# divideon/xvc

Measured on AMD Instinct MI355X. Metric: hot-path frame passes/s (TZ + sub-pel ME, MC, transform + RDOQ + dequant + inverse, deblock, pad, PSNR parts), bit-exact vs the reference's classes, higher is better.
Workload: dtype u16; 1 GPU; 1920x1080 yuv420p 30fps synthetic, QP 32, internal bitdepth 10, 16x16 CUs, TZ range 96, RDOQ (RdoQuant::QuantRdo + CoeffSignHideRdo, picture-initial CABAC contexts); cus_per_picture=8160, parallelism=3 independent picture chains in flight

## Files before the change

### xvc_amd/csrc/k_rdoq.h

```cpp
#ifndef XVCGPU_K_RDOQ_H_
#define XVCGPU_K_RDOQ_H_

#include "dev_common.h"
#include "k_me.h"
#include "k_me2.h"
#include "k_quant.h"
#include "k_rdoq4.h"
#include "k_rdoq_common.h"
#include "k_scan.h"
#include "xvcgpu_internal.h"


template <int G = 64, typename S, typename CF, typename LEV>
__device__ __forceinline__ int wave_rdoq(S &s, int lane, const BlockQuant &bq, int w, int h,
                                         bool luma, int scan_order, bool sign_hide,
                                         const xvcgpu_rdoq_contexts &ctx,
                                         const xvcgpu_rdoq_params &prm, CF cf, LEV lev,
                                         bool stage_ctx = true, bool clear_levels = true) {
  const int sbs = (w == 2 || h == 2) ? 1 : 2;
  const int sb_size = 1 << (2 * sbs);
  const int gw = w >> sbs, gh = h >> sbs;
  const int rw = w < 32 ? w : 32, rh = h < 32 ? h : 32;
  const int rgw = rw >> sbs, rgh = rh >> sbs;
  const int size_cls = (rq_log2(w) + rq_log2(h)) >> 1;
// ... 1307 lines not shown
struct RqGlobalLev {
  int16_t *p;
  int w;
  __device__ __forceinline__ int16_t *operator()(int x, int y) const { return p + y * w + x; }
  __device__ __forceinline__ void store4(int px, int y, const int v[4]) const {
    int16_t *o = p + y * w + px;
    if ((reinterpret_cast<uintptr_t>(o) & 7) == 0) {
      *reinterpret_cast<uint2 *>(o) =
          make_uint2((unsigned)(v[0] & 0xffff) | ((unsigned)v[1] << 16),
                     (unsigned)(v[2] & 0xffff) | ((unsigned)v[3] << 16));
    } else {
      o[0] = (int16_t)v[0]; o[1] = (int16_t)v[1]; o[2] = (int16_t)v[2]; o[3] = (int16_t)v[3];
    }
  }
};

template <int G, int NSB, bool FOUR>
__device__ __forceinline__ void quant_rdo_packed_wave(
    RdoqPackedLds<G, NSB> &sm, int wave, int bd, const xvcgpu_tx_block *blocks, const int *list,
    const int *count, const int16_t *coeffs, const uint32_t *d_off, int16_t *levels,
    int32_t *nnz_out, const xvcgpu_rdoq_contexts *rq_ctx, const xvcgpu_rdoq_params *rq_prm,
    xvcgpu_cu_info *cu_patch = nullptr) {
  constexpr int GROUPS = 64 / G;
  const int g = threadIdx.x / G, lane = threadIdx.x % G;
  const int slot = wave * GROUPS + g;
  RQ_TRACE(0);
  RQ_TRACE_RT(0);
  const int n_list = *count;
  if (wave * GROUPS >= n_list) return;
  const bool active = slot < n_list;
  const int bi = active ? list[slot] : 0;
  const xvcgpu_tx_block b = blocks[bi];
  const xvcgpu_rdoq_params prm = rq_prm[bi];
  const int w = b.w, h = b.h;
  const int rw = w < 32 ? w : 32, rh = h < 32 ? h : 32;
  const uint32_t off = d_off[bi];
  const int16_t *src = coeffs + off;
  int16_t *cf = sm.cf[g], *lv = sm.lv[g];
  constexpr int kCtxWords = (int)sizeof(xvcgpu_rdoq_contexts) / 4;
  const int ctx_wi = (int)threadIdx.x < kCtxWords ? (int)threadIdx.x : kCtxWords - 1;
  const uint32_t word_own = reinterpret_cast<const uint32_t *>(&rq_ctx[prm.ctx_index])[ctx_wi];
  RQ_TRACE(1);
  int16_t *dst = levels + off;
  const bool wide = w == rw && h == rh && ((w * h) & 7) == 0 &&
                    ((reinterpret_cast<uintptr_t>(src) | reinterpret_cast<uintptr_t>(dst)) & 15) == 0;
  const bool sb4 = !(w == 2 || h == 2);
  const int rgw4 = rw >> 2;
  auto tile_pos = [sb4, rgw4, rw](int x, int y) {
    return sb4 ? ((y >> 2) * rgw4 + (x >> 2)) * RQ_CF_STRIDE + (((y & 3) << 2) | (x & 3))
               : y * rw + x;
  };
  if (active) {
    if (wide && sb4) {
      for (int i = lane; i < (w * h) >> 3; i += G) {
        const uint4 v8 = reinterpret_cast<const uint4 *>(src)[i];
        const int y = (8 * i) / rw, x = 8 * i - y * rw;
        const int p0 = tile_pos(x, y), p1 = rw == 4 ? tile_pos(0, y + 1) : tile_pos(x + 4, y);
        *reinterpret_cast<uint2 *>(cf + p0) = make_uint2(v8.x, v8.y);
        *reinterpret_cast<uint2 *>(cf + p1) = make_uint2(v8.z, v8.w);
        if (!FOUR) {
          *reinterpret_cast<uint2 *>(lv + p0) = make_uint2(0, 0);
          *reinterpret_cast<uint2 *>(lv + p1) = make_uint2(0, 0);
        }
      }
    } else {
      for (int i = lane; i < rw * rh; i += G) {
        const int y = i / rw, x = i - y * rw;
        cf[tile_pos(x, y)] = src[y * w + x];
        if (!FOUR) lv[tile_pos(x, y)] = 0;
      }
    }
  }
  RdoqView v;
  v.wl = sm.wl[g];
  v.fcs = NSB == 64 ? sm.fcs : sm.sb_code_cost[g];
  v.sb_dcz = sm.sb_dcz[g];
  v.rate_up = sm.rate_up[g];
  v.sb_live = sm.sb_live[g];
  v.sb_code_cost = sm.sb_code_cost[g];
  v.csbf_bits = sm.csbf_bits[g];
  v.csbf = sm.csbf[g];
  v.sb_of_scan = sm.sb_of_scan[g];
  v.lp_bits = sm.lp_bits;
  v.ctx_bits = sm.ctx_bits;
  RQ_TRACE(2);
  bool pending = active;
  int nnz = 0;
  for (;;) {
    const unsigned long long todo = __ballot(pending);
    if (!todo) break;
    const int leader = __ffsll((long long)todo) - 1;
    const int cur = __shfl((int)prm.ctx_index, leader, 64);
    const int kw = __shfl(w, leader, 64), kh = __shfl(h, leader, 64);
    const int kqp = __shfl((int)b.qp, leader, 64);
    const int kluma = __shfl((int)(b.comp == 0), leader, 64);
    const int kflags = __shfl((int)b.intra_pic, leader, 64);
    const int kpf = __shfl((int)prm.flags, leader, 64);
    const long long klambda = __shfl(prm.lambda, leader, 64);
    wave_sync();
    {
      static_assert(RQ_CTX_WORDS <= 64, "one word of contexts per lane");
      const uint32_t *cw = reinterpret_cast<const uint32_t *>(&rq_ctx[cur]);
      const uint32_t word = (int)prm.ctx_index == cur ? word_own : cw[ctx_wi];
      if ((int)threadIdx.x < RQ_CTX_WORDS)
        rq_stage_word(kEntropyBits, word, sm.ctx_bits + 8 * threadIdx.x);
    }
    wave_sync();
    RQ_TRACE(3);
    const bool take = pending && (int)prm.ctx_index == cur && w == kw && h == kh &&
                      (int)b.qp == kqp && (int)(b.comp == 0) == kluma &&
                      (int)b.intra_pic == kflags && (int)prm.flags == kpf &&
                      prm.lambda == klambda;
    if (take) {
      const int uw = __builtin_amdgcn_readfirstlane(w), uh = __builtin_amdgcn_readfirstlane(h);
      const int uqp = __builtin_amdgcn_readfirstlane((int)b.qp);
      const int uluma = __builtin_amdgcn_readfirstlane((int)(b.comp == 0));
      const int uflags = __builtin_amdgcn_readfirstlane((int)b.intra_pic);
      const int upf = __builtin_amdgcn_readfirstlane((int)prm.flags);
      const unsigned ulam_lo = (unsigned)__builtin_amdgcn_readfirstlane((int)(unsigned)prm.lambda);
      const unsigned ulam_hi = (unsigned)__builtin_amdgcn_readfirstlane(
          (int)(unsigned)((unsigned long long)prm.lambda >> 32));
      const long long ulambda = (long long)(((unsigned long long)ulam_hi << 32) | ulam_lo);
      const bool usb4 = !(uw == 2 || uh == 2);
      const int urw = uw < 32 ? uw : 32, urgw4 = urw >> 2;
      auto utile = [usb4, urgw4, urw](int x, int y) {
        return usb4 ? ((y >> 2) * urgw4 + (x >> 2)) * RQ_CF_STRIDE + (((y & 3) << 2) | (x & 3))
                    : y * urw + x;
      };
      xvcgpu_rdoq_params uprm = prm;
      uprm.lambda = ulambda;
      uprm.flags = (uint8_t)upf;
      const TxBlockFlags ufl = tx_block_flags(uflags);
      const int uscan = ufl.scan_order;
      const bool ush = ufl.sign_hide;
      auto ubq = [&](int bw, int bh) { return block_quant(bw, bh, uqp, bd, ufl.intra_pic); };
      auto cf_at = [cf, utile](int x, int y) { return (int)cf[utile(x, y)]; };
      auto lv_at = [lv, utile](int x, int y) { return lv + utile(x, y); };
      if (FOUR) {
        const RqTileCf cf4 = {cf, urgw4};
        const RqGlobalLev lv4 = {dst, uw};
        nnz = wave_rdoq4<G, 1>(v, lane, ubq(uw, uh), uw, uh, uluma != 0, ush, uprm, cf4, lv4);
      } else if (NSB == 64) {
        const BlockQuant q = ubq(uw, uh);
        if (rq4_takes(64, uw, uh, uscan))
          nnz = wave_rdoq4<64, 4>(v, lane, q, uw, uh, uluma != 0, ush, uprm, cf_at, lv_at);
        else
          nnz = wave_rdoq<G>(v, lane, q, uw, uh, uluma != 0, uscan, ush, rq_ctx[cur], uprm, cf_at,
                             lv_at, false, false);
      } else if (G == 16 && NSB == 16 && uw == 16 && uh == 16) {
        auto cf16 = [cf](int x, int y) {
          return (int)cf[((y >> 2) * 4 + (x >> 2)) * RQ_CF_STRIDE + (((y & 3) << 2) | (x & 3))];
        };
        auto lv16 = [lv](int x, int y) {
          return lv + ((y >> 2) * 4 + (x >> 2)) * RQ_CF_STRIDE + (((y & 3) << 2) | (x & 3));
        };
        nnz = wave_rdoq<G>(v, lane, ubq(16, 16), 16, 16, uluma != 0, uscan, ush, rq_ctx[cur], uprm,
                           cf16, lv16, false, false);
      } else {
        nnz = wave_rdoq<G>(v, lane, ubq(uw, uh), uw, uh, uluma != 0, uscan, ush, rq_ctx[cur], uprm,
                           cf_at, lv_at, false, false);
      }
      pending = false;
    }
  }
  wave_sync();
// ... 89 lines not shown
```

### xvc_amd/csrc/k_rdoq4.h

```cpp
#ifndef XVCGPU_K_RDOQ4_H_
#define XVCGPU_K_RDOQ4_H_

#include "dev_common.h"
#include "k_me2.h"
#include "k_quant.h"
#include "k_rdoq_common.h"
#include "k_scan.h"

template <int I>
__device__ __forceinline__ int rq4_quad_bcast(int v) {
  return __builtin_amdgcn_update_dpp(0, v, I * 0x55, 0xF, 0xF, false);
}
__device__ __forceinline__ int rq4_quad_or(int v) {
  v |= lane_xor<1>(v);
  v |= lane_xor<2>(v);
  return v;
}
__device__ __forceinline__ int rq4_quad_min(int v) {
  int o = lane_xor<1>(v);
  v = o < v ? o : v;
  o = lane_xor<2>(v);
  return o < v ? o : v;
}
__device__ __forceinline__ int rq4_quad_max(int v) {
// ... 26 lines not shown
  }
  return v;
}
template <int G>
__device__ __forceinline__ int rq4_sum(int v) {
  v = dpp_group_sum<16>(v);
  if (G == 64)
    v = __builtin_amdgcn_readlane(v, 0) + __builtin_amdgcn_readlane(v, 16) +
        __builtin_amdgcn_readlane(v, 32) + __builtin_amdgcn_readlane(v, 48);
  return v;
}
template <int G>
__device__ __forceinline__ unsigned rq4_wave_or8(unsigned v, int bits) {
  if (G == 64) {
    int o = rq4_quad_or((int)v);
    o |= rq4_row_half_mirror(o);
    o |= rq4_row_mirror(o);
    return (unsigned)(__builtin_amdgcn_readlane(o, 0) | __builtin_amdgcn_readlane(o, 16) |
                      __builtin_amdgcn_readlane(o, 32) | __builtin_amdgcn_readlane(o, 48));
  }
  unsigned r = 0;
  for (int b = 0; b < bits; b++) r |= (__ballot((v >> b) & 1u) ? 1u : 0u) << b;
  return r;
}
__device__ __forceinline__ long long rq4_readlane_i64(long long v, int l) {
  const unsigned lo = (unsigned)__builtin_amdgcn_readlane((int)(unsigned)v, l);
  const unsigned hi = (unsigned)__builtin_amdgcn_readlane((int)(v >> 32), l);
  return (long long)(((unsigned long long)hi << 32) | lo);
}
__device__ __forceinline__ long long rq4_add_wrap(long long a, long long b) {
  return (long long)((unsigned long long)a + (unsigned long long)b);
}
template <int G>
__device__ __forceinline__ long long rq4_sum_i64(long long v) {
  v = rq_group_sum_i64<16>(v);
  if (G == 64)
    v = rq4_add_wrap(rq4_add_wrap(rq4_readlane_i64(v, 0), rq4_readlane_i64(v, 16)),
                     rq4_add_wrap(rq4_readlane_i64(v, 32), rq4_readlane_i64(v, 48)));
  return v;
}
__device__ __forceinline__ unsigned rq4_row_scan_u32(unsigned v) {
  v += (unsigned)__builtin_amdgcn_update_dpp(0, (int)v, 0x111, 0xF, 0xF, true);
  v += (unsigned)__builtin_amdgcn_update_dpp(0, (int)v, 0x112, 0xF, 0xF, true);
  v += (unsigned)__builtin_amdgcn_update_dpp(0, (int)v, 0x114, 0xF, 0xF, true);
  v += (unsigned)__builtin_amdgcn_update_dpp(0, (int)v, 0x118, 0xF, 0xF, true);
  return v;
}
template <int S>
__device__ __forceinline__ long long rq4_xor_i64(long long v) {
  const int lo = lane_xor<S>((int)(unsigned)v), hi = lane_xor<S>((int)(v >> 32));
  return (long long)(((unsigned long long)(unsigned)hi << 32) | (unsigned)lo);
}
template <int G>
__device__ __forceinline__ long long rq4_suffix_i64(long long v) {
  const long long inc = rq_row_scan_i64(v);
  const long long row = rq_group_sum_i64<16>(v);
  long long behind = rq4_add_wrap(row - inc, v);
  if (G == 64) {
    const long long t1 = rq4_readlane_i64(row, 16), t2 = rq4_readlane_i64(row, 32),
                    t3 = rq4_readlane_i64(row, 48);
    const int r = ME2_LANE >> 4;
    behind = rq4_add_wrap(behind, r == 0 ? rq4_add_wrap(rq4_add_wrap(t1, t2), t3)
                                         : (r == 1 ? rq4_add_wrap(t2, t3) : (r == 2 ? t3 : 0ll)));
  }
  return behind;
}

__device__ __forceinline__ int rq4_sb_scan_index(int gw, int gh, int sx, int sy) {
  const int s = sx + sy, a = gw < gh ? gw : gh, b = gw < gh ? gh : gw;
  int t;
  if (s <= a) {
    t = (s * (s + 1)) >> 1;
  } else if (s <= b) {
    t = ((a * (a + 1)) >> 1) + (s - a) * a;
  } else {
    const int m = gw + gh - 1 - s;
    t = gw * gh - ((m * (m + 1)) >> 1);
  }
  return t + ((s < gh - 1 ? s : gh - 1) - sy);
}

__device__ __forceinline__ bool rq4_takes(int G, int w, int h, int scan_order) {
  const int rw = w < 32 ? w : 32, rh = h < 32 ? h : 32;
  return scan_order == 0 && w >= 4 && h >= 4 && (G == 64 || (rw >> 2) * (rh >> 2) * 4 <= G);
}
__device__ __forceinline__ bool rq4_needs_nr4(int w, int h) {
  const int rw = w < 32 ? w : 32, rh = h < 32 ? h : 32;
  return (rw >> 2) * (rh >> 2) > 16;
}

template <typename CF>
__device__ __forceinline__ auto rq4_load_row(const CF &cf, int px, int y, int c[4])
    -> decltype(cf.row4(px, y, c), void()) {
  cf.row4(px, y, c);
}
template <typename CF, typename... Dummy>
__device__ __forceinline__ void rq4_load_row(const CF &cf, int px, int y, int c[4], Dummy...) {
#pragma unroll
  for (int i = 0; i < 4; i++) c[i] = cf(px + i, y);
}
template <typename LEV>
__device__ __forceinline__ auto rq4_store_row(const LEV &lev, int px, int y, const int v[4])
    -> decltype(lev.store4(px, y, v), void()) {
  lev.store4(px, y, v);
}
template <typename LEV, typename... Dummy>
__device__ __forceinline__ void rq4_store_row(const LEV &lev, int px, int y, const int v[4],
                                              Dummy...) {
#pragma unroll
  for (int i = 0; i < 4; i++) *lev(px + i, y) = (short)v[i];
}
// ... 25 lines not shown
  };
  auto neighbours = [&](int p, int &n_sig, int &n_g1, int &n_g2, int &sum_abs) {
    const int v0 = d_abs((int)wl[p + 1]), v1 = d_abs((int)wl[p + 2]),
              v2 = d_abs((int)wl[p + WS + 1]), v3 = d_abs((int)wl[p + WS]),
              v4 = d_abs((int)wl[p + 2 * WS]);
    n_sig = (v0 != 0) + (v1 != 0) + (v2 != 0) + (v3 != 0) + (v4 != 0);
    n_g1 = (v0 > 1) + (v1 > 1) + (v2 > 1) + (v3 > 1) + (v4 > 1);
    n_g2 = (v0 > 2) + (v1 > 2) + (v2 > 2) + (v3 > 2) + (v4 > 2);
    sum_abs = v0 + v1 + v2 + v3 + v4;
  };
  auto sig_ctx_of = [&](int posxy, int n_sig) {
    return rq_sig_ctx_base(luma, posxy, size_cls) + 2 * (n_sig < 5 ? n_sig : 5);
  };
  auto greater_ctx_nn = [&](int posxy, int nn) { return rq_greater_ctx(luma, posxy, nn); };

  unsigned pa[NR][2], pq[NR][2], negs = 0, valid = 0;
  unsigned sdm = 0;
  int scan_u[NR];
  long long zd_u[NR];
  int last = -1;
  for (int i = lane; i < (WS * (rh + 2)) >> 1; i += G) reinterpret_cast<uint32_t *>(wl)[i] = 0;
  if (outside)
    for (int i = lane; i < 64; i += G) reinterpret_cast<uint32_t *>(s.sb_of_scan)[i] = 0xffffffffu;
#pragma unroll
  for (int r = 0; r < NR; r++) {
    const int sbi = UPR * r + q4i;
    const bool mine = sbi < nsb;
    const int sx = mine ? (sbi & (rgw - 1)) : 0, sy = mine ? (sbi >> lrgw) : 0;
    scan_u[r] = rq4_sb_scan_index(gw, gh, sx, sy);
    int c[4];
    if (mine) rq4_load_row(cf, sx << 2, (sy << 2) + j, c);
    else c[0] = c[1] = c[2] = c[3] = 0;
    unsigned qm = 0;
    unsigned long long sum_sq = 0;
    int a[4], q[4];
#pragma unroll
    for (int i = 0; i < 4; i++) {
      a[i] = (short)d_abs(c[i]);
      q[i] = bq.fwd(a[i]);
      negs |= (unsigned)(c[i] < 0) << (4 * r + i);
      sum_sq += (unsigned)(a[i] * a[i]);
      if (q[i]) {
        qm |= 1u << kof(i);
        if (NR == 1) sdm |= 1u << i;
      }
    }
    pa[r][0] = (unsigned)(a[0] & 0xffff) | ((unsigned)a[1] << 16);
    pa[r][1] = (unsigned)(a[2] & 0xffff) | ((unsigned)a[3] << 16);
    pq[r][0] = (unsigned)(q[0] & 0xffff) | ((unsigned)q[1] << 16);
    pq[r][1] = (unsigned)(q[2] & 0xffff) | ((unsigned)q[3] << 16);
    valid |= (unsigned)mine << r;
    const unsigned qmask = (unsigned)rq4_quad_or((int)qm);
    zd_u[r] = (long long)((unsigned long long)rq_group_sum_i64<4>((long long)sum_sq) << bq.cost_scale);
    const int l = mine && qmask ? (scan_u[r] << 4) + 31 - __clz((int)qmask) : -1;
    last = l > last ? l : last;
  }
  sdm <<= j;
  const int last_pos_index = rq4_max<G>(last);
  RQ_TRACE(4);
  if (last_pos_index < 0) {
#pragma unroll
    for (int r = 0; r < NR; r++)
      if ((valid >> r) & 1u) {
        const int sbi = UPR * r + q4i;
        const int z[4] = {0, 0, 0, 0};
        rq4_store_row(lev, (sbi & (rgw - 1)) << 2, ((sbi >> lrgw) << 2) + j, z);
      }
    return 0;
  }
  auto half = [](const unsigned p[2], int u) {
    const unsigned w2 = u < 2 ? p[0] : p[1];
    return (int)(short)((u & 1) ? (w2 >> 16) : (w2 & 0xffffu));
  };

  const int last_k = last_pos_index & 15, last_sb = last_pos_index >> 4;
  int last_l = -1, d_first = -1;
#pragma unroll
  for (int r = 0; r < NR; r++) {
    const int sbi = UPR * r + q4i;
    const bool mine = (valid >> r) & 1u;
    const bool live = mine && (scan_u[r] << 4) <= last_pos_index;
    if (mine && j == 0) {
      s.sb_of_scan[scan_u[r]] = (unsigned char)sbi;
      s.csbf[sbi] = 0;
      s.sb_dcz[sbi] = 0;
      s.sb_live[sbi] = live ? 1 : 0;
      if (!live) {
        s.csbf_bits[sbi] = 0;
        s.sb_code_cost[sbi] = zd_u[r];
      }
    }
    if (mine && scan_u[r] == last_sb) last_l = sbi;
    const int dd = live ? (sbi & (rgw - 1)) + (sbi >> lrgw) : -1;
    d_first = dd > d_first ? dd : d_first;
  }
  last_l = rq4_max<G>(last_l);
  d_first = rq4_max<G>(d_first);
  constexpr int LPY = 16;
  {
    const int r16 = lane & 15;
    auto axis = [&](bool is_x, int &gmax) {
      gmax = rq_last_pos_group((is_x ? w : h) - 1);
      const bool inr = r16 < gmax;
      const int gc = gmax > 0 ? gmax - 1 : 0;
      const uint2 zb = *reinterpret_cast<const uint2 *>(
          cb + rq_last_pos_ctx(luma, w, h, r16 < gc ? r16 : gc, is_x));
      const unsigned one = inr ? zb.y : 0u, zero = inr ? zb.x : 0u;
      return rq4_row_scan_u32(one) - one + zero +
             (r16 > 3 ? (unsigned)((r16 - 2) >> 1) * RQ_BYPASS : 0u);
    };
    if (G == 64) {
      int gmax;
      const unsigned v = axis(lane < 16, gmax);
      if (lane < 32 && r16 <= gmax) s.lp_bits[(lane < 16 ? 0 : LPY) + r16] = v;
    } else {
      int gx, gy;
      const unsigned vx = axis(true, gx), vy = axis(false, gy);
      if (r16 <= gx) s.lp_bits[r16] = vx;
      if (r16 <= gy) s.lp_bits[LPY + r16] = vy;
    }
  }
  auto sig_pair = [&](unsigned pk, int posxy, int index, int k, bool dcz, unsigned &sig0,
                      unsigned &sig1) {
    const uint2 b2 =
        *reinterpret_cast<const uint2 *>(cb + sig_ctx_of(posxy, (int)((pk >> 12) & 7u)));
    sig0 = b2.x;
    sig1 = (index == last_pos_index || (k == 0 && dcz)) ? 0u : b2.y;
  };
  auto sig_rate_of = [&](unsigned pk, int posxy, int index, int k, bool dcz) {
    if (index >= last_pos_index) return 0;
    unsigned sig0, sig1;
    sig_pair(pk, posxy, index, k, dcz, sig0, sig1);
    return (int)(sig1 - sig0);
  };
  auto state_of = [&](unsigned pk, int posxy, RdoqFlagBits &fb, RdoqCoeffState &st) {
    const uint2 c1_b =
        *reinterpret_cast<const uint2 *>(cb + greater_ctx_nn(posxy, (int)(pk & 7u)));
    const uint2 c2_b =
        *reinterpret_cast<const uint2 *>(cb + greater_ctx_nn(posxy, (int)((pk >> 3) & 7u)));
    fb.c1_0 = c1_b.x; fb.c1_1 = c1_b.y; fb.c2_0 = c2_b.x; fb.c2_1 = c2_b.y;
    st.c1_idx = (pk >> 6) & 1u ? 8 : 0;
    st.c2_idx = (int)((pk >> 7) & 1u);
    st.golomb_rice_k = (pk >> 8) & 15u;
  };
  wave_sync();
  RQ_TRACE(5);

  RQ_STEP_BEGIN();
  for (int d = d_first; d >= 0; d--) {
    int ru = 0;
    bool act = false;
#pragma unroll
    for (int r = 0; r < NR; r++) {
      const int sbi = UPR * r + q4i;
      const bool on = ((valid >> r) & 1u) && (sbi & (rgw - 1)) + (sbi >> lrgw) == d &&
                      (scan_u[r] << 4) <= last_pos_index;
      if (on) {
        ru = r;
        act = true;
      }
    }
    unsigned ua[2], uq[2];
    int my_scan = scan_u[0];
    long long my_zero_dist = zd_u[0];
    ua[0] = pa[0][0]; ua[1] = pa[0][1]; uq[0] = pq[0][0]; uq[1] = pq[0][1];
#pragma unroll
    for (int r = 1; r < NR; r++)
      if (ru == r) {
        ua[0] = pa[r][0]; ua[1] = pa[r][1]; uq[0] = pq[r][0]; uq[1] = pq[r][1];
        my_scan = scan_u[r];
        my_zero_dist = zd_u[r];
      }
    const int sbi = UPR * ru + q4i;
    const int sx = sbi & (rgw - 1), sy = sbi >> lrgw;
    const int sb_index = my_scan << 4;
    const int row_p = ((sy << 2) + j) * WS + (sx << 2);
    RQ_STEP(3);
    int c1 = 0, c2 = 0, nz = 0;
    long long code_cost = 0;
    if (NR > 1)
      sdm = ((unsigned)((uq[0] & 0xffffu) != 0) | ((unsigned)((uq[0] >> 16) != 0) << 1) |
             ((unsigned)((uq[1] & 0xffffu) != 0) << 2) | ((unsigned)((uq[1] >> 16) != 0) << 3)) << j;
    unsigned sds = rq4_wave_or8<G>(act ? sdm : 0u, 7);
    while (sds) {
      const int sd = 31 - __clz((int)sds);
      sds &= ~(1u << sd);
      const int x = sd - j;
      const bool on = act && (unsigned)x < 4u;
      const int xi = on ? x : 0;
      const int qv = half(uq, xi);
      const bool has = on && qv != 0;
      const int abs_coeff = half(ua, xi);
      const int k = kof(xi);
      const int p = row_p + xi;
      const int posxy = 4 * d + sd;
      const int sig_base = rq_sig_ctx_base(luma, posxy, size_cls);
      int nn1 = 0, nn2 = 0, n_sig5 = 0;
      unsigned gr = 0, sig1 = 0;
      RdoqFlagBits fb = {0, 0, 0, 0};
      long long zero_alt = 0, dist_q = 0, dist_q1 = 0;
// ... 59 lines not shown
      };
      unsigned flags = 0;
      int v0 = 0, v1 = 0, v2 = 0, v3 = 0;
      auto settle = [&](auto decide, const bool c2_read) {
        for (;;) {
          if (need) decide();
          const int mylv = has ? best_level : 0;
          int c1t, c2t;
          if (NR == 1) {
            flags = (unsigned)(mylv != 0) | ((unsigned)(mylv >= 1) << 8) | ((unsigned)(mylv >= 2) << 16);
            const unsigned f0 = (unsigned)rq4_quad_bcast<0>((int)flags),
                           f1 = (unsigned)rq4_quad_bcast<1>((int)flags),
                           f2 = (unsigned)rq4_quad_bcast<2>((int)flags);
            const unsigned front = (j > 0 ? f0 : 0u) + (j > 1 ? f1 : 0u) + (j > 2 ? f2 : 0u);
            c1t = c1 + (int)((front >> 8) & 0xffu);
            c2t = c2 + (int)(front >> 16);
          } else {
            v0 = rq4_quad_bcast<0>(mylv);
            v1 = rq4_quad_bcast<1>(mylv);
            v2 = rq4_quad_bcast<2>(mylv);
            v3 = rq4_quad_bcast<3>(mylv);
            c1t = c1 + (j > 0 && v0 >= 1) + (j > 1 && v1 >= 1) + (j > 2 && v2 >= 1);
            c2t = c2 + (j > 0 && v0 >= 2) + (j > 1 && v1 >= 2) + (j > 2 && v2 >= 2);
          }
          need = has && ((c1t < 8) != (c1a < 8) || (c2_read && (c2t < 1) != (c2a < 1)));
          c1a = c1t;
          c2a = c2t;
          if (!__ballot(need)) break;
        }
      };
      if (!__ballot(has && qv != 1)) settle(decide_one, false);
      else settle(decide_any, true);
      if (has) {
        wl[p] = (short)best_level;
        s.rate_up[rec_pos((sx << 2) + xi, (sy << 2) + j)] =
            RQ_STATE_PACK(nn1, nn2, c1a, c2a, gr, n_sig5);
        if (dc_sig_zero) s.sb_dcz[sbi] = 1;
        code_cost += best_cost;
      }
      if (NR == 1) {
        const unsigned quad = (unsigned)dpp_group_sum<4>((int)flags);
        nz += (int)(quad & 0xffu);
        c1 += (int)((quad >> 8) & 0xffu);
        c2 += (int)(quad >> 16);
      } else {
        c1 += (v0 >= 1) + (v1 >= 1) + (v2 >= 1) + (v3 >= 1);
        c2 += (v0 >= 2) + (v1 >= 2) + (v2 >= 2) + (v3 >= 2);
        nz += (v0 != 0) + (v1 != 0) + (v2 != 0) + (v3 != 0);
      }
      wave_sync();
    }
    code_cost = rq_group_sum_i64<4>(code_cost);
    bool any = nz != 0;
    if (act && j == 0) {
      s.sb_code_cost[sbi] = code_cost;
      if (!any && !(sb_index == 0 || sb_index + 16 > last_pos_index)) s.sb_live[sbi] = 4;
    }
    wave_sync();
    RQ_STEP(0);
    {
      const int ax0 = d > rgh - 1 ? d - (rgh - 1) : 0;
      const int ax1 = d < rgw - 1 ? d : rgw - 1;
      const int pairs = (ax1 - ax0 + 1) << 4;
      for (int t0 = 0; t0 < pairs; t0 += G) {
        const int t = t0 + lane;
        const bool in = t < pairs;
        const int ax = ax0 + ((in ? t : 0) >> 4), ay = d - ax, k = t & 15;
        const int l2 = ay * rgw + ax;
        const bool work = in && s.sb_live[l2] == 1;
        if (!__ballot(work)) continue;
        long long cost = 0;
        if (work) {
          const int pp = rq_scan_pos(2, 0, k);
          const int x = (ax << 2) + (pp & 3), y = (ay << 2) + (pp >> 2);
          const int abs_coeff = (short)d_abs(cf(x, y));
          if (!bq.codes(abs_coeff)) {
            cost = bq.zero_dist(abs_coeff);
            if (l2 == last_l && k > last_k) {
              s.rate_up[rec_pos(x, y)] = (unsigned short)RQ_STATE_NO_RATE;
            } else {
              int n_sig, n_g1, n_g2, sum_abs;
              neighbours(y * WS + x, n_sig, n_g1, n_g2, sum_abs);
              cost += rq_bit_cost(cb[sig_ctx_of(x + y, n_sig)], lambda);
              s.rate_up[rec_pos(x, y)] = RQ_STATE_PACK(rq_greater_nn(n_g1, false), 0, 0, 0, 0,
                                                       n_sig < 5 ? n_sig : 5);
            }
          }
        }
        cost = rq_group_sum_i64<16>(cost);
        if ((lane & 15) == 0 && in && cost) s.sb_code_cost[l2] += cost;
      }
    }
    wave_sync();
    RQ_STEP(1);
    bool zeroed = false;
    if (act && j == 0) {
      long long sb_code_cost = s.sb_code_cost[sbi];
      const bool right = sx < rgw - 1 ? s.csbf[sbi + 1] != 0 : false;
      const bool below = sy < rgh - 1 ? s.csbf[sbi + rgw] != 0 : false;
      const int csbf_ctx = 2 * (RQ_OFF(csbf) + (luma ? 0 : 2) + ((right || below) ? 1 : 0));
      unsigned bits_to_zero = 0;
      bool zero_sb = false;
      if (!(sb_index == 0 || sb_index + 16 > last_pos_index)) {
        const unsigned z_bits = cb[csbf_ctx], c_bits = cb[csbf_ctx + 1];
        const long long zero_cost = my_zero_dist + rq_bit_cost(z_bits, lambda);
        if (any) {
          const long long cc = sb_code_cost + rq_bit_cost(c_bits, lambda);
          if (zero_cost < cc) {
            sb_code_cost = zero_cost;
            bits_to_zero = z_bits;
            zero_sb = true;
          } else {
            sb_code_cost = cc;
            bits_to_zero = c_bits;
          }
        } else {
          sb_code_cost = zero_cost;
          bits_to_zero = z_bits;
        }
      }
      if (zero_sb) {
        any = false;
        zeroed = true;
        s.sb_live[sbi] = 2;
      }
      s.csbf[sbi] = any ? 1 : 0;
      s.csbf_bits[sbi] = bits_to_zero;
      s.sb_code_cost[sbi] = sb_code_cost;
    }
    if (__ballot(zeroed)) {
      const bool z = rq4_quad_or((int)zeroed) != 0;
      if (z) {
        wl[row_p] = 0; wl[row_p + 1] = 0; wl[row_p + 2] = 0; wl[row_p + 3] = 0;
      }
    }
    wave_sync();
    RQ_STEP(2);
  }
  RQ_STEP_END();
  long long code_part = 0, zero_part = 0;
#pragma unroll
  for (int r = 0; r < NR; r++)
    if (((valid >> r) & 1u) && j == 0) {
      code_part = rq4_add_wrap(code_part, s.sb_code_cost[UPR * r + q4i]);
      zero_part = rq4_add_wrap(zero_part, zd_u[r]);
    }
  long long comp_code_cost = rq4_sum_i64<G>(code_part);
  const long long comp_zero_dist = rq4_sum_i64<G>(zero_part);
  const unsigned outside_bits = cb[2 * (RQ_OFF(csbf) + (luma ? 0 : 2))];

  RQ_TRACE(6);
  int new_last = 0;
  const int cbf_ctx = 2 * (!luma ? RQ_OFF(cbf_chroma)
                                 : ((prm.flags & XVC_RDOQ_INTRA_CU) ? RQ_OFF(cbf_luma)
                                                                    : RQ_OFF(root_cbf)));
  const long long comp_zero_cost = comp_zero_dist + rq_bit_cost(cb[cbf_ctx], lambda);
  {
    RQ_STEP2_BEGIN();
    int stop_local = -1;
#pragma unroll
    for (int r = 0; r < NR; r++) {
      const int sbi = UPR * r + q4i;
      const bool mine = (valid >> r) & 1u;
      const bool coded = mine && scan_u[r] <= last_sb && s.csbf[mine ? sbi : 0] != 0;
      const int start_k = scan_u[r] == last_sb ? last_k : 15;
      const int rp = mine ? (((sbi >> lrgw) << 2) + j) * WS + ((sbi & (rgw - 1)) << 2) : 0;
      unsigned gt1 = ((unsigned)((int)wl[rp] > 1) << kof(0)) |
                     ((unsigned)((int)wl[rp + 1] > 1) << kof(1)) |
                     ((unsigned)((int)wl[rp + 2] > 1) << kof(2)) |
                     ((unsigned)((int)wl[rp + 3] > 1) << kof(3));
      gt1 = (unsigned)rq4_quad_or((int)gt1) & ((2u << start_k) - 1u);
      const int sl = coded && gt1 ? (scan_u[r] << 4) + 31 - __clz((int)gt1) : -1;
      stop_local = sl > stop_local ? sl : stop_local;
    }
    const int stop_idx = rq4_max<G>(stop_local);
    const int stop_sb = stop_idx >= 0 ? stop_idx >> 4 : 0;
    wave_sync();
    const long long out_cost = rq_bit_cost(outside_bits, lambda);
    constexpr int RND = G == 64 ? 4 : 1;
    unsigned long long todo[RND];
    long long carry = 0;
    int n_out = 0;
#pragma unroll
    for (int rr = RND - 1; rr >= 0; rr--) {
      todo[rr] = 0;
      if (rr * G > last_sb) continue;
      const int kk = rr * G + lane;
      const bool inw = kk <= last_sb && (outside || kk < nsb);
      const int tj = inw ? (outside ? (int)s.sb_of_scan[kk] : (int)s.sb_of_scan[kk]) : 255;
      const bool corner = inw && (!outside || tj != 255);
      long long fc = 0;
      if (corner) fc = rq_bit_cost(s.csbf_bits[tj], lambda);
      const bool outc = inw && !corner && kk > 0 && kk < last_sb;
      if (outc) fc = out_cost;
      const bool cd = corner && kk >= stop_sb && s.csbf[corner ? tj : 0] != 0;
      const long long behind = rq4_add_wrap(rq4_suffix_i64<G>(fc), carry);
      if (inw) fcs[kk] = behind;
      if (G == 64) {
        carry = rq4_readlane_i64(behind, 0);
        todo[rr] = __ballot(cd);
        n_out += __popcll(__ballot(outc));
      } else {
        todo[rr] = (__ballot(cd) >> (ME2_LANE & 48)) & 0xffffull;
      }
    }
    comp_code_cost = rq4_add_wrap(comp_code_cost, (long long)n_out * out_cost);
    wave_sync();
    RQ_STEP(0);
    const int kk = lane & 15;
    const int p16 = rq_scan_pos(2, 0, kk);
    const long long base = comp_code_cost + rq_bit_cost(cb[cbf_ctx + 1], lambda);
    long long best_cost = 0x7fffffffffffffffll;
    int best_last_plus1 = 0;
    long long acc = 0;
    for (;;) {
      int jj = -1;
      if (G == 64) {
        int pick[4] = {-1, -1, -1, -1};
        int n = 0;
#pragma unroll
        for (int rr = RND - 1; rr >= 0; rr--)
          while (n < 4 && todo[rr]) {
            const int b = 63 - __clzll((long long)todo[rr]);
            todo[rr] &= ~(1ull << b);
            pick[n++] = rr * 64 + b;
          }
        if (n == 0) break;
        const int row = lane >> 4;
        jj = row == 0 ? pick[0] : (row == 1 ? pick[1] : (row == 2 ? pick[2] : pick[3]));
      } else {
        if (!__ballot(todo[0] != 0)) break;
        if (todo[0]) {
          jj = 63 - __clzll((long long)todo[0]);
          todo[0] &= ~(1ull << jj);
        }
      }
      const bool on = jj >= 0;
      const int js = on ? jj : 0;
      const int t = on ? (int)s.sb_of_scan[js] : 0;
      const long long flags_behind = fcs[js];
      const bool dcz = s.sb_dcz[t] != 0;
      const int x = ((t & (rgw - 1)) << 2) + (p16 & 3), y = ((t >> lrgw) << 2) + (p16 >> 2);
      const int index = (js << 4) + kk;
      const int first_k = js == last_sb ? last_k : 15;
      const bool in = on && kk <= first_k && index >= stop_idx;
      const unsigned pk = (unsigned)s.rate_up[rec_pos(x, y)];
      const int v = (int)wl[y * WS + x];
      const int ac = (short)d_abs(cf(x, y));
      unsigned sig0, sig1;
      sig_pair(pk, x + y, index, kk, dcz, sig0, sig1);
      long long ctz = 0;
      if (in && index != stop_idx) {
        ctz = -rq_bit_cost(sig0, lambda);
        if (v == 1) {
          const unsigned c1_0 = cb[greater_ctx_nn(x + y, (int)(pk & 7u))];
          const unsigned bits1 = sig1 + (((pk >> 6) & 1u) ? (2u + ((pk >> 8) & 15u)) * RQ_BYPASS
                                                         : RQ_BYPASS + c1_0);
          ctz = bq.zero_dist(ac) - (bq.dist(ac - bq.dequant(1)) + rq_bit_cost(bits1, lambda));
        } else if (v < 0) {
          ctz = bq.zero_dist(ac) - 0x7fffffffffffffffll;
        }
      }
      const long long inc = rq_row_scan_i64(ctz);
      const long long total = rq_group_sum_i64<16>(ctz);
      long long acc_row = acc;
      if (G == 64) {
        const long long t0 = rq4_readlane_i64(total, 0), t1 = rq4_readlane_i64(total, 16),
                        t2 = rq4_readlane_i64(total, 32), t3 = rq4_readlane_i64(total, 48);
        const int row = lane >> 4;
        const long long t01 = rq4_add_wrap(t0, t1), t012 = rq4_add_wrap(t01, t2);
        acc_row = rq4_add_wrap(acc_row, row == 0 ? 0ll : (row == 1 ? t0 : (row == 2 ? t01 : t012)));
        acc = rq4_add_wrap(acc, rq4_add_wrap(t012, t3));
      } else {
        acc = rq4_add_wrap(acc, total);
      }
      if (in && v != 0) {
        const unsigned lp_bits = s.lp_bits[rq_last_pos_group(x)] +
                                 s.lp_bits[LPY + rq_last_pos_group(y)];
        const long long cost = base - flags_behind + acc_row + (total - inc) +
                               rq_bit_cost(lp_bits, lambda) - rq_bit_cost(sig1, lambda);
        if (cost < best_cost) {
          best_cost = cost;
          best_last_plus1 = index + 1;
        }
      }
    }
    RQ_STEP(1);
    auto keep_better = [&](long long oc, int oi) {
      if (oc < best_cost || (oc == best_cost && oi > best_last_plus1)) {
        best_cost = oc;
        best_last_plus1 = oi;
      }
    };
    keep_better(rq4_xor_i64<1>(best_cost), lane_xor<1>(best_last_plus1));
    keep_better(rq4_xor_i64<2>(best_cost), lane_xor<2>(best_last_plus1));
    {
      const int lo = rq4_row_half_mirror((int)(unsigned)best_cost),
                hi = rq4_row_half_mirror((int)(best_cost >> 32));
      keep_better((long long)(((unsigned long long)(unsigned)hi << 32) | (unsigned)lo),
                  rq4_row_half_mirror(best_last_plus1));
    }
    {
      const int lo = rq4_row_mirror((int)(unsigned)best_cost),
                hi = rq4_row_mirror((int)(best_cost >> 32));
      keep_better((long long)(((unsigned long long)(unsigned)hi << 32) | (unsigned)lo),
                  rq4_row_mirror(best_last_plus1));
    }
    if (G == 64) {
      const long long c0 = rq4_readlane_i64(best_cost, 0), c1r = rq4_readlane_i64(best_cost, 16),
                      c2r = rq4_readlane_i64(best_cost, 32), c3 = rq4_readlane_i64(best_cost, 48);
      const int i0 = __builtin_amdgcn_readlane(best_last_plus1, 0),
                i1 = __builtin_amdgcn_readlane(best_last_plus1, 16),
                i2 = __builtin_amdgcn_readlane(best_last_plus1, 32),
                i3 = __builtin_amdgcn_readlane(best_last_plus1, 48);
      best_cost = c0;
      best_last_plus1 = i0;
      keep_better(c1r, i1);
      keep_better(c2r, i2);
      keep_better(c3, i3);
    }
    new_last = comp_zero_cost < best_cost ? -1 : best_last_plus1;
    RQ_STEP(3);
    RQ_STEP2_END();
  }

  RQ_TRACE(7);
  int nnz = 0;
  unsigned has_sb = 0;
  unsigned pl[NR][2];
#pragma unroll
  for (int r = 0; r < NR; r++) {
    const int sbi = UPR * r + q4i;
    const bool mine = (valid >> r) & 1u;
    const int sx = sbi & (rgw - 1), sy = sbi >> lrgw;
    const int rp = mine ? ((sy << 2) + j) * WS + (sx << 2) : 0;
    int lvv[4] = {(int)wl[rp], (int)wl[rp + 1], (int)wl[rp + 2], (int)wl[rp + 3]};
    int cnt = 0;
#pragma unroll
    for (int i = 0; i < 4; i++) {
      int level = lvv[i];
      if (new_last < 0 || (scan_u[r] << 4) + kof(i) >= new_last) level = 0;
      cnt += level != 0;
      lvv[i] = (short)((negs >> (4 * r + i)) & 1u ? -level : level);
    }
    if (!mine) cnt = 0;
    if (mine) rq4_store_row(lev, sx << 2, (sy << 2) + j, lvv);
    pl[r][0] = (unsigned)(lvv[0] & 0xffff) | ((unsigned)lvv[1] << 16);
    pl[r][1] = (unsigned)(lvv[2] & 0xffff) | ((unsigned)lvv[3] << 16);
    has_sb |= (unsigned)(rq4_quad_or(cnt) != 0) << r;
    nnz += cnt;
  }
  nnz = rq4_sum<G>(nnz);
  if (new_last < 0) return 0;
  if (!(sign_hide && nnz > 1)) return nnz;

  RQ_TRACE(8);
  int lss = -1;
#pragma unroll
  for (int r = 0; r < NR; r++)
    if (((has_sb >> r) & 1u) && scan_u[r] > lss) lss = scan_u[r];
  const int last_sb_scan = rq4_max<G>(lss);
  int dn = 0;
#pragma unroll
  for (int r = 0; r < NR; r++) {
    const int sbi = UPR * r + q4i;
    const int sx = sbi & (rgw - 1), sy = sbi >> lrgw;
    const int sb_index = scan_u[r] << 4;
    int lv4[4] = {half(pl[r], 0), half(pl[r], 1), half(pl[r], 2), half(pl[r], 3)};
    int first = 16, lastk = -1, sum = 0;
#pragma unroll
    for (int i = 0; i < 4; i++)
      if (lv4[i]) {
        const int k = kof(i);
        first = k < first ? k : first;
        lastk = k > lastk ? k : lastk;
        sum += lv4[i];
      }
    first = rq4_quad_min(first);
// ... 89 lines not shown
```

### xvc_amd/csrc/k_rdoq_common.h

```cpp
#ifndef XVCGPU_K_RDOQ_COMMON_H_
#define XVCGPU_K_RDOQ_COMMON_H_

#include "dev_common.h"
#include "k_me.h"
#include "k_me2.h"
#include "k_quant.h"
#include "k_scan.h"
#include "xvcgpu_internal.h"

#ifdef XVCGPU_TRACE
__device__ unsigned long long g_rq_trace[4096][16];
#define RQ_TRACE(k)                                                          \
  do {                                                                       \
    if (threadIdx.x == 0 && blockIdx.x < 4096)                               \
      g_rq_trace[blockIdx.x][k] = __builtin_amdgcn_s_memtime();              \
  } while (0)
#define RQ_TRACE_RT(k)                                                       \
  do {                                                                       \
    if (threadIdx.x == 0 && blockIdx.x < 2048)                               \
      g_rq_trace[2048 + blockIdx.x][k] = __builtin_amdgcn_s_memrealtime();   \
  } while (0)
#else
#define RQ_TRACE(k) do {} while (0)
#define RQ_TRACE_RT(k) do {} while (0)
#endif
#ifdef XVCGPU_TRACE
#define RQ_STEP_BEGIN() unsigned long long rq_t_ = __builtin_amdgcn_s_memtime(), rq_a_[4] = {0, 0, 0, 0}
#define RQ_STEP(i)                                              \
  do {                                                          \
    const unsigned long long n_ = __builtin_amdgcn_s_memtime(); \
    rq_a_[i] += n_ - rq_t_;                                     \
    rq_t_ = n_;                                                 \
  } while (0)
#define RQ_STEP_END()                                                           \
  do {                                                                          \
    if (threadIdx.x == 0 && blockIdx.x < 2048)                                  \
      for (int i_ = 0; i_ < 4; i_++) g_rq_trace[blockIdx.x][11 + i_] = rq_a_[i_]; \
  } while (0)
#define RQ_STEP2_BEGIN() rq_t_ = __builtin_amdgcn_s_memtime(); rq_a_[0] = rq_a_[1] = rq_a_[2] = rq_a_[3] = 0
#define RQ_STEP2_END()                                                          \
  do {                                                                          \
    if (threadIdx.x == 0 && blockIdx.x < 2048)                                  \
      for (int i_ = 0; i_ < 4; i_++) g_rq_trace[2048 + blockIdx.x][11 + i_] = rq_a_[i_]; \
  } while (0)
#else
#define RQ_STEP_BEGIN() do {} while (0)
#define RQ_STEP(i) do {} while (0)
#define RQ_STEP_END() do {} while (0)
#define RQ_STEP2_BEGIN() do {} while (0)
#define RQ_STEP2_END() do {} while (0)
#endif

#define RQ_SB_STRIDE 17
#define RQ_PADDED(n) ((n) + (n) / 16)
#define RQ_CF_STRIDE 20
#define RQ_CF_PADDED(n) ((n) + (n) / 4)

#define RQ_WL(n) ((n) + 2 * ((n) >= 1024 ? 64 : ((n) >= 256 ? 40 : 20)) + 4)

template <int N0>
struct RdoqShared {
  static constexpr int N = RQ_PADDED(N0);
  unsigned short rate_up[N];
  long long sb_code_cost[64];
  unsigned csbf_bits[64];
  unsigned char csbf[64];
  unsigned char sb_live[64];
  unsigned char sb_dcz[64];
  unsigned char sb_of_scan[256];
  unsigned lp_bits[32];
  alignas(8) unsigned ctx_bits[2 * sizeof(xvcgpu_rdoq_contexts)];
  alignas(8) int16_t wl[RQ_WL(N0)];
  long long fcs_store[N0 >= 1024 ? 256 : 1];
};
template <int N0>
__device__ __forceinline__ long long *rq_fcs(RdoqShared<N0> &s) {
  return N0 >= 1024 ? s.fcs_store : s.sb_code_cost;
}

struct RdoqView {
  int16_t *wl;
  long long *fcs;
  unsigned short *rate_up;
  long long *sb_code_cost;
  unsigned *csbf_bits;
  unsigned char *csbf, *sb_live, *sb_dcz;
  unsigned char *sb_of_scan;
  unsigned *lp_bits;
  unsigned *ctx_bits;
};

__device__ __forceinline__ int rq_last_pos_group(int pos) {
  if (pos < 4) return pos;
  const int l = 31 - __clz(pos);
  return 2 * l + ((pos >> (l - 1)) & 1);
}
template <int G>
__device__ __forceinline__ int rq_wave_max_i32(int v) {
// ... 142 lines not shown
```

Baseline: 9916 frame passes/s.

## Trim RDOQ wave reductions and skip empty-diagonal pricing passes

Several micro-optimizations in the wave-level RDOQ kernel. The last-position index and its subgroup are packed into one value so one max reduction replaces three. The per-diagonal rate pricing pass is skipped when no subgroup needs pricing, and for single-row cases the CSBF zeroing decision is deferred past the loop. Suffix and prefix scans, plus the best-last reduction, avoid cross-row work when only one row is in use. The single-group path uses readfirstlane instead of leader shuffles, and a division becomes a shift. Trace counters are added under the debug flag. Bit-exactness depends on the deferred CSBF path and the packed encoding (which assumes at most 64 subblocks) matching the original ordering.

```diff
diff --git a/xvc_amd/csrc/k_rdoq.h b/xvc_amd/csrc/k_rdoq.h
--- a/xvc_amd/csrc/k_rdoq.h
+++ b/xvc_amd/csrc/k_rdoq.h
@@ -1383,9 +1383,10 @@
   };
   if (active) {
     if (wide && sb4) {
+      const int lrw = FOUR ? rq_log2(rw) : 0;
       for (int i = lane; i < (w * h) >> 3; i += G) {
         const uint4 v8 = reinterpret_cast<const uint4 *>(src)[i];
-        const int y = (8 * i) / rw, x = 8 * i - y * rw;
+        const int y = FOUR ? (8 * i) >> lrw : (8 * i) / rw, x = 8 * i - y * rw;
         const int p0 = tile_pos(x, y), p1 = rw == 4 ? tile_pos(0, y + 1) : tile_pos(x + 4, y);
         *reinterpret_cast<uint2 *>(cf + p0) = make_uint2(v8.x, v8.y);
         *reinterpret_cast<uint2 *>(cf + p1) = make_uint2(v8.z, v8.w);
@@ -1420,14 +1421,24 @@
   for (;;) {
     const unsigned long long todo = __ballot(pending);
     if (!todo) break;
-    const int leader = __ffsll((long long)todo) - 1;
-    const int cur = __shfl((int)prm.ctx_index, leader, 64);
-    const int kw = __shfl(w, leader, 64), kh = __shfl(h, leader, 64);
-    const int kqp = __shfl((int)b.qp, leader, 64);
-    const int kluma = __shfl((int)(b.comp == 0), leader, 64);
-    const int kflags = __shfl((int)b.intra_pic, leader, 64);
-    const int kpf = __shfl((int)prm.flags, leader, 64);
-    const long long klambda = __shfl(prm.lambda, leader, 64);
+    int cur;
+    bool same;
+    if (GROUPS == 1) {
+      cur = __builtin_amdgcn_readfirstlane((int)prm.ctx_index);
+      same = true;
+    } else {
+      const int leader = __ffsll((long long)todo) - 1;
+      cur = __shfl((int)prm.ctx_index, leader, 64);
+      const int kw = __shfl(w, leader, 64), kh = __shfl(h, leader, 64);
+      const int kqp = __shfl((int)b.qp, leader, 64);
+      const int kluma = __shfl((int)(b.comp == 0), leader, 64);
+      const int kflags = __shfl((int)b.intra_pic, leader, 64);
+      const int kpf = __shfl((int)prm.flags, leader, 64);
+      const long long klambda = __shfl(prm.lambda, leader, 64);
+      same = (int)prm.ctx_index == cur && w == kw && h == kh && (int)b.qp == kqp &&
+             (int)(b.comp == 0) == kluma && (int)b.intra_pic == kflags && (int)prm.flags == kpf &&
+             prm.lambda == klambda;
+    }
     wave_sync();
     {
       static_assert(RQ_CTX_WORDS <= 64, "one word of contexts per lane");
@@ -1438,10 +1449,7 @@
     }
     wave_sync();
     RQ_TRACE(3);
-    const bool take = pending && (int)prm.ctx_index == cur && w == kw && h == kh &&
-                      (int)b.qp == kqp && (int)(b.comp == 0) == kluma &&
-                      (int)b.intra_pic == kflags && (int)prm.flags == kpf &&
-                      prm.lambda == klambda;
+    const bool take = pending && same;
     if (take) {
       const int uw = __builtin_amdgcn_readfirstlane(w), uh = __builtin_amdgcn_readfirstlane(h);
       const int uqp = __builtin_amdgcn_readfirstlane((int)b.qp);
diff --git a/xvc_amd/csrc/k_rdoq4.h b/xvc_amd/csrc/k_rdoq4.h
--- a/xvc_amd/csrc/k_rdoq4.h
+++ b/xvc_amd/csrc/k_rdoq4.h
@@ -102,11 +102,11 @@
   return (long long)(((unsigned long long)(unsigned)hi << 32) | (unsigned)lo);
 }
 template <int G>
-__device__ __forceinline__ long long rq4_suffix_i64(long long v) {
+__device__ __forceinline__ long long rq4_suffix_i64(long long v, bool one_row = false) {
   const long long inc = rq_row_scan_i64(v);
   const long long row = rq_group_sum_i64<16>(v);
   long long behind = rq4_add_wrap(row - inc, v);
-  if (G == 64) {
+  if (G == 64 && !one_row) {
     const long long t1 = rq4_readlane_i64(row, 16), t2 = rq4_readlane_i64(row, 32),
                     t3 = rq4_readlane_i64(row, 48);
     const int r = ME2_LANE >> 4;
@@ -238,11 +238,12 @@
     valid |= (unsigned)mine << r;
     const unsigned qmask = (unsigned)rq4_quad_or((int)qm);
     zd_u[r] = (long long)((unsigned long long)rq_group_sum_i64<4>((long long)sum_sq) << bq.cost_scale);
-    const int l = mine && qmask ? (scan_u[r] << 4) + 31 - __clz((int)qmask) : -1;
+    const int l = mine && qmask ? ((((scan_u[r] << 4) + 31 - __clz((int)qmask)) << 6) | sbi) : -1;
     last = l > last ? l : last;
   }
   sdm <<= j;
-  const int last_pos_index = rq4_max<G>(last);
+  const int last_packed = rq4_max<G>(last);
+  const int last_pos_index = last_packed >> 6;
   RQ_TRACE(4);
   if (last_pos_index < 0) {
 #pragma unroll
@@ -260,7 +261,8 @@
   };
 
   const int last_k = last_pos_index & 15, last_sb = last_pos_index >> 4;
-  int last_l = -1, d_first = -1;
+  const int last_l = last_packed & 63;
+  const int d_first = (last_l & (rgw - 1)) + (last_l >> lrgw);
 #pragma unroll
   for (int r = 0; r < NR; r++) {
     const int sbi = UPR * r + q4i;
@@ -276,12 +278,7 @@
         s.sb_code_cost[sbi] = zd_u[r];
       }
     }
-    if (mine && scan_u[r] == last_sb) last_l = sbi;
-    const int dd = live ? (sbi & (rgw - 1)) + (sbi >> lrgw) : -1;
-    d_first = dd > d_first ? dd : d_first;
-  }
-  last_l = rq4_max<G>(last_l);
-  d_first = rq4_max<G>(d_first);
+  }
   constexpr int LPY = 16;
   {
     const int r16 = lane & 15;
@@ -332,6 +329,9 @@
   wave_sync();
   RQ_TRACE(5);
 
+  bool deferred = false;
+  RQ_COUNTS();
+  RQ_COUNT(0, d_first + 1);
   RQ_STEP_BEGIN();
   for (int d = d_first; d >= 0; d--) {
     int ru = 0;
@@ -497,13 +497,16 @@
     }
     code_cost = rq_group_sum_i64<4>(code_cost);
     bool any = nz != 0;
+    const bool priced = act && (any || sb_index == 0 || sb_index + 16 > last_pos_index);
     if (act && j == 0) {
       s.sb_code_cost[sbi] = code_cost;
       if (!any && !(sb_index == 0 || sb_index + 16 > last_pos_index)) s.sb_live[sbi] = 4;
     }
     wave_sync();
     RQ_STEP(0);
-    {
+    RQ_COUNT(2, __ballot(priced) != 0);
+    RQ_COUNT(3, __popcll(__ballot(priced && j == 0)));
+    if (__ballot(priced)) {
       const int ax0 = d > rgh - 1 ? d - (rgh - 1) : 0;
       const int ax1 = d < rgw - 1 ? d : rgw - 1;
       const int pairs = (ax1 - ax0 + 1) << 4;
@@ -515,6 +518,9 @@
         const bool work = in && s.sb_live[l2] == 1;
         if (!__ballot(work)) continue;
         long long cost = 0;
+#ifdef XVCGPU_TRACE
+        bool rq_rated = false, rq_empty = false;
+#endif
         if (work) {
           const int pp = rq_scan_pos(2, 0, k);
           const int x = (ax << 2) + (pp & 3), y = (ay << 2) + (pp >> 2);
@@ -529,9 +535,17 @@
               cost += rq_bit_cost(cb[sig_ctx_of(x + y, n_sig)], lambda);
               s.rate_up[rec_pos(x, y)] = RQ_STATE_PACK(rq_greater_nn(n_g1, false), 0, 0, 0, 0,
                                                        n_sig < 5 ? n_sig : 5);
+#ifdef XVCGPU_TRACE
+              rq_rated = true;
+              rq_empty = n_sig == 0;
+#endif
             }
           }
         }
+#ifdef XVCGPU_TRACE
+        RQ_COUNT(4, __popcll(__ballot(rq_rated)));
+        RQ_COUNT(5, __popcll(__ballot(rq_empty)));
+#endif
         cost = rq_group_sum_i64<16>(cost);
         if ((lane & 15) == 0 && in && cost) s.sb_code_cost[l2] += cost;
       }
@@ -539,7 +553,10 @@
     wave_sync();
     RQ_STEP(1);
     bool zeroed = false;
-    if (act && j == 0) {
+    const bool defer = NR == 1 && !__ballot(act && any);
+    if (defer) deferred = deferred || act;
+    RQ_COUNT(1, !__ballot(act && any));
+    if (!defer && act && j == 0) {
       long long sb_code_cost = s.sb_code_cost[sbi];
       const bool right = sx < rgw - 1 ? s.csbf[sbi + 1] != 0 : false;
       const bool below = sy < rgh - 1 ? s.csbf[sbi + rgw] != 0 : false;
@@ -573,7 +590,7 @@
       s.csbf_bits[sbi] = bits_to_zero;
       s.sb_code_cost[sbi] = sb_code_cost;
     }
-    if (__ballot(zeroed)) {
+    if (!defer && __ballot(zeroed)) {
       const bool z = rq4_quad_or((int)zeroed) != 0;
       if (z) {
         wl[row_p] = 0; wl[row_p + 1] = 0; wl[row_p + 2] = 0; wl[row_p + 3] = 0;
@@ -583,6 +600,20 @@
     RQ_STEP(2);
   }
   RQ_STEP_END();
+  if (NR == 1 && __ballot(deferred)) {
+    if (deferred && j == 0) {
+      const int sx = q4i & (rgw - 1), sy = q4i >> lrgw, sb_index = scan_u[0] << 4;
+      unsigned bits_to_zero = 0;
+      if (!(sb_index == 0 || sb_index + 16 > last_pos_index)) {
+        const bool right = sx < rgw - 1 ? s.csbf[q4i + 1] != 0 : false;
+        const bool below = sy < rgh - 1 ? s.csbf[q4i + rgw] != 0 : false;
+        bits_to_zero = cb[2 * (RQ_OFF(csbf) + (luma ? 0 : 2) + ((right || below) ? 1 : 0))];
+        s.sb_code_cost[q4i] = zd_u[0] + rq_bit_cost(bits_to_zero, lambda);
+      }
+      s.csbf_bits[q4i] = bits_to_zero;
+    }
+    wave_sync();
+  }
   long long code_part = 0, zero_part = 0;
 #pragma unroll
   for (int r = 0; r < NR; r++)
@@ -622,7 +653,8 @@
     const int stop_sb = stop_idx >= 0 ? stop_idx >> 4 : 0;
     wave_sync();
     const long long out_cost = rq_bit_cost(outside_bits, lambda);
-    constexpr int RND = G == 64 ? 4 : 1;
+    constexpr int RND = (G == 64 && NR > 1) ? 4 : 1;
+    const bool one_row = G == 64 && NR == 1 && last_sb < 16;
     unsigned long long todo[RND];
     long long carry = 0;
     int n_out = 0;
@@ -639,7 +671,7 @@
       const bool outc = inw && !corner && kk > 0 && kk < last_sb;
       if (outc) fc = out_cost;
       const bool cd = corner && kk >= stop_sb && s.csbf[corner ? tj : 0] != 0;
-      const long long behind = rq4_add_wrap(rq4_suffix_i64<G>(fc), carry);
+      const long long behind = rq4_add_wrap(rq4_suffix_i64<G>(fc, one_row), carry);
       if (inw) fcs[kk] = behind;
       if (G == 64) {
         carry = rq4_readlane_i64(behind, 0);
@@ -658,6 +690,7 @@
     long long best_cost = 0x7fffffffffffffffll;
     int best_last_plus1 = 0;
     long long acc = 0;
+    int rows_used = 0;
     for (;;) {
       int jj = -1;
       if (G == 64) {
@@ -671,6 +704,9 @@
             pick[n++] = rr * 64 + b;
           }
         if (n == 0) break;
+        rows_used = n > rows_used ? n : rows_used;
+        RQ_COUNT(6, n);
+        RQ_COUNT(7, 1);
         const int row = lane >> 4;
         jj = row == 0 ? pick[0] : (row == 1 ? pick[1] : (row == 2 ? pick[2] : pick[3]));
       } else {
@@ -707,22 +743,23 @@
         }
       }
       const long long inc = rq_row_scan_i64(ctz);
-      const long long total = rq_group_sum_i64<16>(ctz);
-      long long acc_row = acc;
+      long long upto;
       if (G == 64) {
-        const long long t0 = rq4_readlane_i64(total, 0), t1 = rq4_readlane_i64(total, 16),
-                        t2 = rq4_readlane_i64(total, 32), t3 = rq4_readlane_i64(total, 48);
+        const long long t0 = rq4_readlane_i64(inc, 15), t1 = rq4_readlane_i64(inc, 31),
+                        t2 = rq4_readlane_i64(inc, 47), t3 = rq4_readlane_i64(inc, 63);
         const int row = lane >> 4;
-        const long long t01 = rq4_add_wrap(t0, t1), t012 = rq4_add_wrap(t01, t2);
-        acc_row = rq4_add_wrap(acc_row, row == 0 ? 0ll : (row == 1 ? t0 : (row == 2 ? t01 : t012)));
-        acc = rq4_add_wrap(acc, rq4_add_wrap(t012, t3));
+        const long long t01 = rq4_add_wrap(t0, t1), t012 = rq4_add_wrap(t01, t2),
+                        t0123 = rq4_add_wrap(t012, t3);
+        upto = rq4_add_wrap(acc, row == 0 ? t0 : (row == 1 ? t01 : (row == 2 ? t012 : t0123)));
+        acc = rq4_add_wrap(acc, t0123);
       } else {
-        acc = rq4_add_wrap(acc, total);
+        acc = rq4_add_wrap(acc, rq_group_sum_i64<16>(ctz));
+        upto = acc;
       }
       if (in && v != 0) {
         const unsigned lp_bits = s.lp_bits[rq_last_pos_group(x)] +
                                  s.lp_bits[LPY + rq_last_pos_group(y)];
-        const long long cost = base - flags_behind + acc_row + (total - inc) +
+        const long long cost = base - flags_behind + (upto - inc) +
                                rq_bit_cost(lp_bits, lambda) - rq_bit_cost(sig1, lambda);
         if (cost < best_cost) {
           best_cost = cost;
@@ -752,23 +789,31 @@
                   rq4_row_mirror(best_last_plus1));
     }
     if (G == 64) {
-      const long long c0 = rq4_readlane_i64(best_cost, 0), c1r = rq4_readlane_i64(best_cost, 16),
-                      c2r = rq4_readlane_i64(best_cost, 32), c3 = rq4_readlane_i64(best_cost, 48);
-      const int i0 = __builtin_amdgcn_readlane(best_last_plus1, 0),
-                i1 = __builtin_amdgcn_readlane(best_last_plus1, 16),
-                i2 = __builtin_amdgcn_readlane(best_last_plus1, 32),
-                i3 = __builtin_amdgcn_readlane(best_last_plus1, 48);
-      best_cost = c0;
-      best_last_plus1 = i0;
-      keep_better(c1r, i1);
-      keep_better(c2r, i2);
-      keep_better(c3, i3);
+      const long long c0 = rq4_readlane_i64(best_cost, 0);
+      const int i0 = __builtin_amdgcn_readlane(best_last_plus1, 0);
+      if (rows_used > 1) {
+        const long long c1r = rq4_readlane_i64(best_cost, 16), c2r = rq4_readlane_i64(best_cost, 32),
+                        c3 = rq4_readlane_i64(best_cost, 48);
+        const int i1 = __builtin_amdgcn_readlane(best_last_plus1, 16),
+                  i2 = __builtin_amdgcn_readlane(best_last_plus1, 32),
+                  i3 = __builtin_amdgcn_readlane(best_last_plus1, 48);
+        best_cost = c0;
+        best_last_plus1 = i0;
+        keep_better(c1r, i1);
+        keep_better(c2r, i2);
+        keep_better(c3, i3);
+      } else {
+        best_cost = c0;
+        best_last_plus1 = i0;
+      }
     }
     new_last = comp_zero_cost < best_cost ? -1 : best_last_plus1;
     RQ_STEP(3);
     RQ_STEP2_END();
   }
 
+  RQ_COUNT(8, last_sb >= G);
+  RQ_COUNTS_END();
   RQ_TRACE(7);
   int nnz = 0;
   unsigned has_sb = 0;
diff --git a/xvc_amd/csrc/k_rdoq_common.h b/xvc_amd/csrc/k_rdoq_common.h
--- a/xvc_amd/csrc/k_rdoq_common.h
+++ b/xvc_amd/csrc/k_rdoq_common.h
@@ -12,7 +12,7 @@
 __device__ unsigned long long g_rq_trace[4096][16];
 #define RQ_TRACE(k)                                                          \
   do {                                                                       \
-    if (threadIdx.x == 0 && blockIdx.x < 4096)                               \
+    if (threadIdx.x == 0 && blockIdx.x < 2048)    \
       g_rq_trace[blockIdx.x][k] = __builtin_amdgcn_s_memtime();              \
   } while (0)
 #define RQ_TRACE_RT(k)                                                       \
@@ -43,7 +43,17 @@
     if (threadIdx.x == 0 && blockIdx.x < 2048)                                  \
       for (int i_ = 0; i_ < 4; i_++) g_rq_trace[2048 + blockIdx.x][11 + i_] = rq_a_[i_]; \
   } while (0)
+#define RQ_COUNTS() unsigned long long rq_n_[9] = {0, 0, 0, 0, 0, 0, 0, 0, 0}
+#define RQ_COUNT(i, v) (rq_n_[i] += (unsigned long long)(v))
+#define RQ_COUNTS_END()                                                         \
+  do {                                                                          \
+    if (threadIdx.x == 0 && blockIdx.x < 2048)                                  \
+      for (int i_ = 0; i_ < 9; i_++) g_rq_trace[2048 + blockIdx.x][2 + i_] = rq_n_[i_]; \
+  } while (0)
 #else
+#define RQ_COUNTS() do {} while (0)
+#define RQ_COUNT(i, v) do {} while (0)
+#define RQ_COUNTS_END() do {} while (0)
 #define RQ_STEP_BEGIN() do {} while (0)
 #define RQ_STEP(i) do {} while (0)
 #define RQ_STEP_END() do {} while (0)
```

After: 10000 frame passes/s, median of 6. No clear change (+0.8%).
